# NVIDIA-Genomics-Research/GenomeWorks

Measured on AMD Instinct MI355X. Metric: cudapoa consensus GCUPS, 1024-window short-read batch (static band 256, 32 reads <= 1024 bp), higher is better.
Workload: dtype int16; 1 GPU; BASELINE configs[2]: cudapoa single-batch consensus, 1024 windows x 32 reads, backbone 960 bp, <=48 sub/24 ins/24 del, BatchConfig(1024,32,256,static_band), scores 8/-6/-8; windows_per_gpu=1024, cells_per_gpu=10990578176, parallelism=index-split x1

## Files before the change

genomeworks_amd/build.py:

```python
import hashlib
import os
import subprocess
import sys

PKG = os.path.dirname(os.path.abspath(__file__))
ROOT = os.path.dirname(PKG)
LIB = os.path.join(PKG, "lib")
ROCM = os.environ.get("ROCM_PATH", "/opt/rocm")
HIPCC = os.path.join(ROCM, "bin", "hipcc")

KERNEL_SRCS = ["csrc/gwhip_poa.hip", "csrc/gwhip_poa_part0.hip", "csrc/gwhip_poa_part1.hip", "csrc/gwhip_poa_part2.hip",
               "csrc/gwhip_poa_part3.hip", "csrc/gwhip_poa_part4.hip", "csrc/gwhip_poa_part5.hip", "csrc/gwhip_poa_part6.hip", "csrc/gwhip_poa_part7.hip", "csrc/gwhip_poa_hooks.hip", "csrc/gwhip_myers.hip", "csrc/gwhip_ukkonen.hip"]
HOST_SRCS = ["host/capi.cpp", "host/cudapoa_batch.cpp", "host/cudapoa_utils.cpp", "host/cudaaligner.cpp", "host/aligner_global.cpp", "host/device_pool.cpp",
             "host/aligner_semiglobal.cpp", "host/alignment_impl.cpp", "host/runtime.cpp", "host/logging.cpp", "host/overlap_alignment.cpp", "host/multi_device.cpp",
             "host/fasta_parser.cpp"]
EXTENDER_KERNEL_SRCS = ["extender/gwx_ungapped_xdrop.hip"]
EXTENDER_HOST_SRCS = ["extender/extender.cpp"]
SEMIGLOBAL_KERNEL_SRCS = ["semiglobal/gws_ends.hip"]
MAPPER_KERNEL_SRCS = ["mapper/gwm_mapper.hip", "mapper/gwm_postprocess.hip", "mapper/gwm_align.hip",
                      "mapper/gwm_index_cache.hip"]
MAPPER_HOST_SRCS = ["mapper/mapper.cpp", "mapper/gwm_driver.cpp", "mapper/gwm_index_batcher.cpp"]

KERNEL_FLAGS = ["--offload-arch=gfx950", "-O3", "-std=c++17", "-fPIC", "-fno-fast-math", "-ffp-contract=off",
                "-fhip-fp32-correctly-rounded-divide-sqrt"]
KERNEL_FLAGS += [f for f in os.environ.get("GW_KERNEL_EXTRA_FLAGS", "").split() if f]
HOST_FLAGS = ["-O2", "-g", "-std=c++17", "-fPIC", "-Wall", "-Wextra", "-Wno-unused-parameter",
              "-D__HIP_PLATFORM_AMD__", "-pthread"]


def _digest(paths, extra):
    h = hashlib.sha256(repr(extra).encode())
    for p in sorted(paths):
        with open(p, "rb") as f:
            h.update(p.encode())
            h.update(f.read())
    return h.hexdigest()


def kernel_source_digest():
    h = hashlib.sha256()
    base = os.path.join(PKG, "csrc")
    paths = [os.path.join(base, f) for f in os.listdir(base) if f.endswith((".hip", ".h"))] + [os.path.join(ROOT, "include", "gwhip.h")]
    for p in sorted(paths):
        with open(p, "rb") as f:
            h.update(os.path.relpath(p, ROOT).encode())
            h.update(f.read())
    return h.hexdigest()


def _deps(subdir, exts):
    out = []
    for base in (os.path.join(PKG, subdir), os.path.join(ROOT, "include")):
        for d, _, fs in os.walk(base):
            out += [os.path.join(d, f) for f in fs if f.endswith(exts)]
    return out


def _run(cmd):
    print("[build]", " ".join(cmd), flush=True)
    subprocess.run(cmd, check=True)


def _stale(target, stamp_value):
    stamp = target + ".stamp"
    if not os.path.exists(target) or not os.path.exists(stamp):
# ... 161 lines not shown
```

genomeworks_amd/csrc/gwhip_poa.hip:

```cpp
#include <hip/hip_runtime.h>

#include <cstdio>
#include <cstdlib>
#include <cstring>
#include <string>

#include "poa_device.h"
#include "poa_full_device.h"
#include "poa_graph_device.h"
#include "poa_tb_device.h"

namespace gwhip
{

#ifndef GWHIP_POA_PART
thread_local std::string g_last_error;

static int fail(hipError_t e, const char* what)
{
    g_last_error = std::string(what) + ": " + hipGetErrorString(e);
    return (int)e;
}
static int fail_msg(int code, const std::string& msg)
{
    g_last_error = msg;
    return code;
}
#endif

constexpr int kRingBytes   = 8448;
constexpr int kRowInfoLds  = 3074;
constexpr int kRowInfoBytes = kRowInfoLds * 8;
constexpr int kReadLds     = 2048;
constexpr int kCodeTileLds = 4096;
static_assert(kReadLds + kCodeTileLds >= 3072 * 2, "the incremental topsort keeps the previous order (uint16 x 3072) in the read + code-tile regions");
constexpr int kBsRingBytes   = 2048;
constexpr int kReadWinBytes  = 4096;
constexpr int kMwLds         = 768;
constexpr size_t kReservedCuLds = 128 * 1024;

struct KernelArgs
{
    gwhip_poa_config cfg;
    PoaLayout L;
    int32_t total_windows;
    const uint8_t* sequences;
    const int8_t* base_weights;
    int32_t* sequence_lengths;
    const gwhip_window_details* window_details;
    uint8_t* consensus;
    uint16_t* coverage;
    uint8_t* msa;
    uint8_t* workspace;
    uint8_t* full_scores;
    uint64_t* cells;
    uint64_t* phase_cycles;
    int32_t debug_flags;
    int32_t cons_lds_nodes;
    int32_t wide_ring_bytes;
    uint32_t* work_counters;
};

template <typename IdT>
__device__ GraphView<IdT> carve_graph(uint8_t* slab, const PoaLayout& L)
{
    GraphView<IdT> g;
    g.nodes                = slab + L.nodes;
    g.incoming_edge_count  = (uint16_t*)(slab + L.in_cnt);
    g.outgoing_edge_count  = (uint16_t*)(slab + L.out_cnt);
    g.node_alignment_count = (uint16_t*)(slab + L.aln_cnt);
    g.coverage             = (uint16_t*)(slab + L.coverage);
    g.sorted_poa           = (IdT*)(slab + L.sorted);
    g.node_id_to_pos       = (IdT*)(slab + L.pos);
    g.local_cnt            = (uint16_t*)(slab + L.local_cnt);
    g.incoming_edges       = (IdT*)(slab + L.in_edges);
    g.incoming_edge_w      = (uint16_t*)(slab + L.in_w);
    g.outgoing_edges       = (IdT*)(slab + L.out_edges);
    g.node_alignments      = (IdT*)(slab + L.aligned);
    g.cons_scores          = (int32_t*)(slab + L.cons_scores);
    g.cons_pred            = (IdT*)(slab + L.cons_pred);
    g.marks                = slab + L.marks;
    g.check                = slab + L.check;
    g.to_visit             = (IdT*)(slab + L.to_visit);
    g.out_cov              = (uint16_t*)(slab + L.out_cov);
    g.out_cov_cnt          = (uint16_t*)(slab + L.out_cov_cnt);
    g.msa_pos              = (IdT*)(slab + L.msa_pos);
    g.seq_begin            = (IdT*)(slab + L.seq_begin);
    return g;
}

template <typename ScoreT, typename IdT, typename TraceT, int BM, bool MSA, bool LDS_TABLES, int NW, int VARIANT>
__global__ __launch_bounds__(kWave * NW) void poa_window_kernel(KernelArgs a)
{
    constexpr bool DBG = VARIANT == 1 || VARIANT == 4 || VARIANT == 6;
    constexpr int PV   = VARIANT == 0 ? 0 : (VARIANT <= 2 ? 1 : 2);
    constexpr bool kFullPacked = (VARIANT == 5 || VARIANT == 6) && BM == GWHIP_FULL_BAND && LDS_TABLES && std::is_same<ScoreT, int16_t>::value;
    const int32_t debug_flags = DBG ? a.debug_flags : 0;
    extern __shared__ __attribute__((aligned(16))) uint8_t smem[];
    const int lane       = threadIdx.x & (kWave - 1);
    const int wave       = __builtin_amdgcn_readfirstlane((int)threadIdx.x >> 6);
    for (int32_t w = blockIdx.x; w < a.total_windows;)
    {
    const gwhip_poa_config& c = a.cfg;
    uint8_t* slab        = a.workspace + (size_t)w * a.L.per_window;
    GraphView<IdT> g     = carve_graph<IdT>(slab, a.L);
    const gwhip_window_details wd = a.window_details[w];
    int32_t* seq_lens    = a.sequence_lengths + wd.seq_len_buffer_offset;
    const uint8_t* sequence    = a.sequences + wd.seq_starts;
    const int8_t* base_weights = a.base_weights + wd.seq_starts;
    uint8_t* consensus   = a.consensus + (size_t)w * c.max_consensus_size;
    int32_t* alignment_graph = (int32_t*)(slab + a.L.align_graph);
    int32_t* alignment_read  = (int32_t*)(slab + a.L.align_read);

    ScoreT* ring = reinterpret_cast<ScoreT*>(smem);
    uint8_t* lds_rowinfo_region = smem + kRingBytes;
    uint8_t* lds_read_buf       = smem + kRingBytes + kRowInfoBytes;
    uint8_t* lds_code_tile      = LDS_TABLES ? smem + kRingBytes + kRowInfoBytes + kReadLds : nullptr;
    const int32_t ring_bytes    = LDS_TABLES ? kRingBytes : a.wide_ring_bytes;
    int32_t* lds_bs_ring        = LDS_TABLES ? nullptr : reinterpret_cast<int32_t*>(smem + ring_bytes);
    uint8_t* lds_read_window    = LDS_TABLES ? nullptr : smem + ring_bytes + kBsRingBytes;
    uint8_t* codes              = a.L.codes ? slab + a.L.codes : nullptr;
    constexpr bool graph_fits_lds = LDS_TABLES;
    using RowT = RowInfo<LDS_TABLES>;
    RowT* rowinfo;
    if constexpr (LDS_TABLES)
        rowinfo = reinterpret_cast<RowT*>(smem + kRingBytes);
    else
        rowinfo = reinterpret_cast<RowT*>(slab + a.L.rowinfo);

    constexpr bool TB = (BM == GWHIP_STATIC_BAND_TRACEBACK || BM == GWHIP_ADAPTIVE_BAND_TRACEBACK);
    ScoreT* scores;
    uint8_t* full_moves = nullptr;
    if (BM == GWHIP_FULL_BAND)
    {
        const size_t cell_bytes = sizeof(ScoreT) + (sizeof(ScoreT) == 2 ? 1 : 0);
        uint8_t* region         = a.full_scores + (size_t)wd.scores_offset * (size_t)c.max_nodes_per_graph * cell_bytes;
        scores                  = reinterpret_cast<ScoreT*>(region);
        if (sizeof(ScoreT) == 2) full_moves = region + (size_t)wd.scores_width * (size_t)c.max_nodes_per_graph * sizeof(ScoreT);
    }
    else
        scores = reinterpret_cast<ScoreT*>(slab + a.L.scores);
    TraceT* traceback = TB ? reinterpret_cast<TraceT*>(slab + a.L.trace) : nullptr;
    const float banded_buffer_size = __fmul_rn((float)c.max_nodes_per_graph, (float)c.matrix_sequence_dimension);
    MwArgs<ScoreT>* mw_args = nullptr;
    MwShared* mw_shared     = nullptr;
    if constexpr (NW > 1)
    {
        {
            int32_t bases = lane < (int32_t)wd.num_seqs ? seq_lens[lane] : 0;
            for (int off = 32; off > 0; off >>= 1) bases += __shfl_xor(bases, off);
            bases = __builtin_amdgcn_readfirstlane(bases);
            const int32_t level = bases >= (1 << 19) ? 3 : (bases >= (1 << 18) ? 2 : (bases >= (1 << 17) ? 1 : 0));
            if (level == 3) __builtin_amdgcn_s_setprio(3);
            else if (level == 2) __builtin_amdgcn_s_setprio(2);
            else if (level == 1) __builtin_amdgcn_s_setprio(1);
// ... 239 lines not shown
        if constexpr (kCachedSort)
        {
            const bool incr_ok = c.max_nodes_per_graph <= 131071 && !(debug_flags & (1 << 17)) &&
                                 (int64_t)a.L.scores_elems * (int64_t)sizeof(ScoreT) >= (int64_t)c.max_nodes_per_graph * 24 + 2048;
            if (status_and_count >= 0 && !c.spoa_accurate && !(debug_flags & (1 << 21)) && incr_ok)
            {
                wave_sync();
                bool done = false;
                if (!(debug_flags & (1 << 16)) && topsort_incr_cnt8_lds_bytes(status_and_count) <= ring_bytes)
                    done = topsort_kahn_incr_cnt8<IdT>(g, node_count, status_and_count, smem, reinterpret_cast<int32_t*>(scores), lane);
                if (!done) topsort_kahn_incr_hbm<IdT>(g, node_count, status_and_count, reinterpret_cast<int32_t*>(scores), lane);
                sorted_here = true;
            }
            else if (status_and_count >= 0 && !c.spoa_accurate && !(debug_flags & (1 << 21)) &&
                     (int64_t)a.L.scores_elems * (int64_t)sizeof(ScoreT) >= (int64_t)(2 * ((node_count + 63) & ~63)) * 4)
            {
                wave_sync();
                topsort_kahn_cached<IdT>(g, node_count, status_and_count, smem, reinterpret_cast<int32_t*>(scores), lane);
                sorted_here = true;
            }
        }
        if (lane == 0 && status_and_count >= 0 && !sorted_here)
        {
            const int32_t new_count = status_and_count;
            if (c.spoa_accurate)
                topsort_racon<IdT>(g, new_count, (int32_t)(uint16_t)c.max_nodes_per_graph);
            else if (!graph_fits_lds)
                topsort_kahn<IdT>(g.sorted_poa, g.node_id_to_pos, new_count, g.incoming_edge_count,
                                  g.outgoing_edges, g.outgoing_edge_count, g.local_cnt);
        }
        wave_sync();
        if (status_and_count >= 0 && !c.spoa_accurate && graph_fits_lds)
        {
            if constexpr (LDS_TABLES)
            {
                if (!(debug_flags & (1 << 21)))
                    topsort_kahn_incr_lds<IdT>(g, node_count, status_and_count, lds_rowinfo_region, smem, lds_read_buf, lane,
                                               debug_flags, pc.acc ? &pc.acc[kPhOther] : nullptr);
                else
                    topsort_kahn_lds<IdT>(g, status_and_count, lds_rowinfo_region, smem, lane, debug_flags, pc.acc ? &pc.acc[kPhOther] : nullptr);
            }
        }
        pc.tick(kPhTopsort);
        if (status_and_count < 0) break;
        node_count = status_and_count;
    }
    if (lane == 0 && a.cells) a.cells[w] = cells;
    if (DBG && lane == 0 && a.phase_cycles)
        for (int k = 0; k < kPhCount; k++) a.phase_cycles[(size_t)w * kPhCount + k] = phase_acc[k];
    if constexpr (NW > 1)
    {
        if (lane == 0) mw_args->op = 2;
        block_barrier();
        break;
    }
    else
    {
        if ((int32_t)gridDim.x >= a.total_windows || a.work_counters == nullptr) break;
        wave_sync();
        int32_t next = 0;
        if (lane == 0) next = (int32_t)gridDim.x + (int32_t)atomicAdd(a.work_counters, 1u);
        w = wave_first(next);
    }
    }
    if constexpr (NW == 1)
        if ((int32_t)gridDim.x < a.total_windows && a.work_counters != nullptr && threadIdx.x == 0)
        {
            __threadfence();
            if (atomicAdd(a.work_counters + 1, 1u) == gridDim.x - 1)
            {
                a.work_counters[0] = 0;
                a.work_counters[1] = 0;
                __threadfence();
            }
        }
}

#ifndef GWHIP_POA_PART
template <typename IdT>
__global__ __launch_bounds__(kWave) void poa_consensus_kernel(KernelArgs a)
{
    const int32_t w    = blockIdx.x;
    const gwhip_poa_config& c = a.cfg;
    uint8_t* consensus = a.consensus + (size_t)w * c.max_consensus_size;
    if (consensus[0] == kKernelError) return;
    uint8_t* slab      = a.workspace + (size_t)w * a.L.per_window;
    GraphView<IdT> g   = carve_graph<IdT>(slab, a.L);
    const int32_t n    = a.sequence_lengths[a.window_details[w].seq_len_buffer_offset];
    if (threadIdx.x == 0)
        generate_consensus<IdT>(g, n, g.cons_pred, g.cons_scores, consensus, a.coverage + (size_t)w * c.max_consensus_size,
                                c.max_consensus_size);
}

__global__ __launch_bounds__(kWave) void poa_consensus_lds_kernel(KernelArgs a)
{
    extern __shared__ __align__(16) uint8_t cons_smem[];
    const int32_t w    = blockIdx.x;
    const gwhip_poa_config& c = a.cfg;
    uint8_t* consensus = a.consensus + (size_t)w * c.max_consensus_size;
    if (consensus[0] == kKernelError) return;
    uint8_t* slab          = a.workspace + (size_t)w * a.L.per_window;
    GraphView<int16_t> g   = carve_graph<int16_t>(slab, a.L);
    const int32_t n        = a.sequence_lengths[a.window_details[w].seq_len_buffer_offset];
    if (n <= a.cons_lds_nodes)
        generate_consensus_lds<int16_t>(g, n, cons_smem, a.cons_lds_nodes, consensus, a.coverage + (size_t)w * c.max_consensus_size,
                                        c.max_consensus_size, threadIdx.x & (kWave - 1),
                                        (a.debug_flags & 16) != 0);
    else if (threadIdx.x == 0)
        generate_consensus<int16_t>(g, n, g.cons_pred, g.cons_scores, consensus, a.coverage + (size_t)w * c.max_consensus_size,
                                    c.max_consensus_size);
}

constexpr int kMsaStackEntries = 4096;

template <typename IdT>
__global__ __launch_bounds__(kWave) void poa_msa_kernel(KernelArgs a)
{
    extern __shared__ __attribute__((aligned(16))) uint8_t msa_smem[];
    __shared__ int32_t msa_length;
    const int32_t w    = blockIdx.x;
    const gwhip_poa_config& c = a.cfg;
    uint8_t* consensus = a.consensus + (size_t)w * c.max_consensus_size;
    if (consensus[0] == kKernelError) return;
    uint8_t* slab      = a.workspace + (size_t)w * a.L.per_window;
    GraphView<IdT> g   = carve_graph<IdT>(slab, a.L);
    const gwhip_window_details wd = a.window_details[w];
    const int32_t n    = a.sequence_lengths[wd.seq_len_buffer_offset];
    const int lane     = threadIdx.x & (kWave - 1);
// ... 35 lines not shown
__global__ void poa_export_graph_kernel(KernelArgs a, int32_t first_window, uint8_t* nodes, int32_t* in_edges, uint16_t* in_w,
                                        uint16_t* in_cnt, int32_t* out_edges, uint16_t* out_cnt)
{
    const int32_t w  = first_window + blockIdx.x;
    const size_t o   = blockIdx.x;
    const int32_t mn = a.cfg.max_nodes_per_graph;
    uint8_t* slab    = a.workspace + (size_t)w * a.L.per_window;
    GraphView<IdT> g = carve_graph<IdT>(slab, a.L);
    const int32_t n  = a.sequence_lengths[a.window_details[w].seq_len_buffer_offset];
    if (a.consensus[(size_t)w * a.cfg.max_consensus_size] == kKernelError) return;
    for (int32_t i = threadIdx.x; i < n && i < mn; i += blockDim.x)
    {
        nodes[o * mn + i]  = g.nodes[i];
        uint16_t ic        = g.incoming_edge_count[i];
        in_cnt[o * mn + i] = ic;
        for (int32_t e = 0; e < ic && e < kEdges; e++)
        {
            in_edges[(o * mn + i) * kEdges + e] = g.incoming_edges[(int64_t)i * kEdges + e];
            in_w[(o * mn + i) * kEdges + e]     = g.incoming_edge_w[(int64_t)i * kEdges + e];
        }
        if (out_edges && out_cnt)
        {
            uint16_t oc         = g.outgoing_edge_count[i];
            out_cnt[o * mn + i] = oc;
            for (int32_t e = 0; e < oc && e < kEdges; e++)
                out_edges[(o * mn + i) * kEdges + e] = g.outgoing_edges[(int64_t)i * kEdges + e];
        }
    }
}

#endif

#ifndef GWHIP_DEVICE_ONLY
#ifndef GWHIP_POA_PART
static size_t full_score_bytes(const gwhip_poa_config& c, int32_t windows, uint64_t sum_scores_width)
{
    if (c.band_mode != GWHIP_FULL_BAND) return 0;
    uint64_t per_window_width = (uint64_t)((c.max_sequence_size + 1 + kCellsPerLane + 3) & ~3);
    uint64_t width_sum        = sum_scores_width ? sum_scores_width : per_window_width * (uint64_t)windows;
    return (size_t)(width_sum * (uint64_t)c.max_nodes_per_graph * (c.score32 ? 4u : 3u)) + 256;
}

static bool validate(const gwhip_poa_args* args)
{
    const gwhip_poa_config& c = args->cfg;
    if (args->total_windows < 0 || c.max_nodes_per_graph <= 0 || c.max_consensus_size < 2) return false;
    if (c.band_mode < 0 || c.band_mode > GWHIP_ADAPTIVE_BAND_TRACEBACK) return false;
    if (c.band_mode != GWHIP_FULL_BAND && (c.alignment_band_width % 128 != 0 || c.alignment_band_width <= 0)) return false;
    if (!c.size32 && c.max_nodes_per_graph > 32767) return false;
    return true;
}
#endif

template <int BM, bool MSA, int VARIANT>
hipError_t launch_packed_variant(const KernelArgs& ka, dim3 grid, size_t lds, hipStream_t stream);
#if defined(GWHIP_POA_PART) && GWHIP_POA_PART >= 4
template <int BM, bool MSA, int VARIANT>
hipError_t launch_packed_variant(const KernelArgs& ka, dim3 grid, size_t lds, hipStream_t stream)
{
    hipLaunchKernelGGL((poa_window_kernel<int16_t, int16_t, int8_t, BM, MSA, true, 1, VARIANT>), grid, dim3(kWave), lds, stream, ka);
    return hipGetLastError();
}
#if GWHIP_POA_PART == 7
template hipError_t launch_packed_variant<GWHIP_FULL_BAND, false, 5>(const KernelArgs&, dim3, size_t, hipStream_t);
template hipError_t launch_packed_variant<GWHIP_FULL_BAND, true, 5>(const KernelArgs&, dim3, size_t, hipStream_t);
template hipError_t launch_packed_variant<GWHIP_FULL_BAND, false, 6>(const KernelArgs&, dim3, size_t, hipStream_t);
template hipError_t launch_packed_variant<GWHIP_FULL_BAND, true, 6>(const KernelArgs&, dim3, size_t, hipStream_t);
#elif GWHIP_POA_PART == 4 || GWHIP_POA_PART == 5
#if GWHIP_POA_PART == 4
#define GW_PACKED_VARIANTS(BM, MSA) template hipError_t launch_packed_variant<BM, MSA, 2>(const KernelArgs&, dim3, size_t, hipStream_t);
#else
#define GW_PACKED_VARIANTS(BM, MSA)                                                                       \
    template hipError_t launch_packed_variant<BM, MSA, 3>(const KernelArgs&, dim3, size_t, hipStream_t); \
    template hipError_t launch_packed_variant<BM, MSA, 4>(const KernelArgs&, dim3, size_t, hipStream_t);
#endif
GW_PACKED_VARIANTS(GWHIP_STATIC_BAND, false)
GW_PACKED_VARIANTS(GWHIP_STATIC_BAND, true)
GW_PACKED_VARIANTS(GWHIP_ADAPTIVE_BAND, false)
GW_PACKED_VARIANTS(GWHIP_ADAPTIVE_BAND, true)
#undef GW_PACKED_VARIANTS
#endif
#endif

template <typename ScoreT, typename IdT, typename TraceT, bool MSA, bool LDS_TABLES>
static hipError_t launch_window_kernel(const KernelArgs& ka_in, hipStream_t stream)
{
    KernelArgs ka = ka_in;
    constexpr size_t wide_rest = (size_t)kBsRingBytes + kReadWinBytes + kMwLds;
    ka.wide_ring_bytes = 5 * (kMaxAdaptiveBand + kRightPad) * 4;
    const size_t lds   = LDS_TABLES ? (size_t)kRingBytes + kRowInfoBytes + kReadLds + kCodeTileLds : (size_t)ka.wide_ring_bytes + wide_rest;
    dim3 grid(ka.total_windows);
    if (LDS_TABLES && ka.work_counters != nullptr)
    {
        static const int simds = [] {
            int cus = 0, dev = 0;
            (void)hipGetDevice(&dev);
            if (hipDeviceGetAttribute(&cus, hipDeviceAttributeMultiprocessorCount, dev) != hipSuccess || cus <= 0) cus = 256;
            return 4 * cus;
        }();
        if (ka.total_windows > simds) grid = dim3(simds);
    }
    if (grid.x >= (unsigned)ka.total_windows) ka.work_counters = nullptr;
#define GW_LAUNCH(BM)                                                                                              \
    {                                                                                                              \
        constexpr int NW = (!LDS_TABLES && BM == GWHIP_ADAPTIVE_BAND) ? kSkWaves : 1;                              \
        size_t lds_req = lds;                                                                                      \
        if (NW > 1)              \
        {                                                                                                          \
            lds_req            = kReservedCuLds;                                                                   \
            ka.wide_ring_bytes = (int32_t)(kReservedCuLds - wide_rest);                                            \
            (void)hipFuncSetAttribute(reinterpret_cast<const void*>(&poa_window_kernel<ScoreT, IdT, TraceT, BM, MSA, LDS_TABLES, NW, 0>), \
                                      hipFuncAttributeMaxDynamicSharedMemorySize, (int)kReservedCuLds);             \
            (void)hipFuncSetAttribute(reinterpret_cast<const void*>(&poa_window_kernel<ScoreT, IdT, TraceT, BM, MSA, LDS_TABLES, NW, 1>), \
                                      hipFuncAttributeMaxDynamicSharedMemorySize, (int)kReservedCuLds);             \
        }                                                                                                          \
        constexpr bool kHasPacked = LDS_TABLES && std::is_same<ScoreT, int16_t>::value && std::is_same<TraceT, int8_t>::value && \
                                    (BM == GWHIP_STATIC_BAND || BM == GWHIP_ADAPTIVE_BAND);                        \
        const bool debug = ka.debug_flags != 0 || ka.phase_cycles != nullptr;                                      \
        const int32_t bw = ka.cfg.alignment_band_width;                                                            \
        bool launched    = false;                                                                                  \
        if constexpr (kHasPacked)                                                                                  \
        {                                                                                                          \
            constexpr int PBM = kHasPacked ? BM : GWHIP_STATIC_BAND;                                               \
            if (bw == 384 || bw == 512)                                                                            \
            {                                                                                                      \
                hipError_t pe = debug ? launch_packed_variant<PBM, MSA, 4>(ka, grid, lds_req, stream)             \
                                      : launch_packed_variant<PBM, MSA, 3>(ka, grid, lds_req, stream);            \
                if (pe != hipSuccess) return pe;                                                                   \
                launched = true;                                                                                   \
            }                                                                                                      \
            else if (bw == 128 && !debug)                                                                          \
            {                                                                                                      \
                hipError_t pe = launch_packed_variant<PBM, MSA, 2>(ka, grid, lds_req, stream);                     \
                if (pe != hipSuccess) return pe;                                                                   \
                launched = true;                                                                                   \
            }                                                                                                      \
        }                                                                                                          \
        if constexpr (BM == GWHIP_FULL_BAND && LDS_TABLES && std::is_same<ScoreT, int16_t>::value && std::is_same<IdT, int16_t>::value && \
                      std::is_same<TraceT, int8_t>::value)                                                         \
        {                                                                                                          \
            hipError_t pe = debug ? launch_packed_variant<GWHIP_FULL_BAND, MSA, 6>(ka, grid, lds_req, stream)      \
                                  : launch_packed_variant<GWHIP_FULL_BAND, MSA, 5>(ka, grid, lds_req, stream);     \
            if (pe != hipSuccess) return pe;                                                                       \
            launched = true;                                                                                       \
        }                                                                                                          \
        if (launched) {}                                                                                           \
        else if (debug)                                                                                            \
            hipLaunchKernelGGL((poa_window_kernel<ScoreT, IdT, TraceT, BM, MSA, LDS_TABLES, NW, 1>), grid, dim3(kWave * NW), lds_req, stream, ka); \
        else                                                                                                       \
            hipLaunchKernelGGL((poa_window_kernel<ScoreT, IdT, TraceT, BM, MSA, LDS_TABLES, NW, 0>), grid, dim3(kWave * NW), lds_req, stream, ka); \
    }                                                                                                              \
    break;
    switch (ka.cfg.band_mode)
    {
    case GWHIP_FULL_BAND: GW_LAUNCH(GWHIP_FULL_BAND)
    case GWHIP_STATIC_BAND: GW_LAUNCH(GWHIP_STATIC_BAND)
    case GWHIP_ADAPTIVE_BAND: GW_LAUNCH(GWHIP_ADAPTIVE_BAND)
    case GWHIP_STATIC_BAND_TRACEBACK: GW_LAUNCH(GWHIP_STATIC_BAND_TRACEBACK)
    default: GW_LAUNCH(GWHIP_ADAPTIVE_BAND_TRACEBACK)
    }
#undef GW_LAUNCH
    return hipGetLastError();
}

template <typename ScoreT, typename IdT, typename TraceT>
hipError_t launch_msa_split(const KernelArgs& ka, hipStream_t stream)
{
    constexpr bool can_lds = sizeof(IdT) == 2;
    const bool lds = can_lds && ka.cfg.max_nodes_per_graph + 2 <= kRowInfoLds && ka.cfg.max_sequence_size + 16 <= kReadLds;
    if (ka.cfg.output_mask & 2)
    {
        if constexpr (can_lds)
            if (lds) return launch_window_kernel<ScoreT, IdT, TraceT, true, true>(ka, stream);
        return launch_window_kernel<ScoreT, IdT, TraceT, true, false>(ka, stream);
    }
    if constexpr (can_lds)
        if (lds) return launch_window_kernel<ScoreT, IdT, TraceT, false, true>(ka, stream);
    return launch_window_kernel<ScoreT, IdT, TraceT, false, false>(ka, stream);
}

#if defined(GWHIP_POA_PART) && GWHIP_POA_PART == 6
template hipError_t launch_msa_split<int16_t, int16_t, int16_t>(const KernelArgs&, hipStream_t);
#else
extern template hipError_t launch_msa_split<int16_t, int16_t, int16_t>(const KernelArgs&, hipStream_t);
#endif

template <typename ScoreT, typename IdT>
hipError_t launch_trace_split(const KernelArgs& ka, hipStream_t stream)
{
    const bool tb = ka.cfg.band_mode == GWHIP_STATIC_BAND_TRACEBACK || ka.cfg.band_mode == GWHIP_ADAPTIVE_BAND_TRACEBACK;
    if (tb && ka.cfg.trace16) return launch_msa_split<ScoreT, IdT, int16_t>(ka, stream);
    return launch_msa_split<ScoreT, IdT, int8_t>(ka, stream);
}
#ifdef GWHIP_POA_PART
#if GWHIP_POA_PART == 0
template hipError_t launch_trace_split<int32_t, int32_t>(const KernelArgs&, hipStream_t);
#elif GWHIP_POA_PART == 1
template hipError_t launch_trace_split<int32_t, int16_t>(const KernelArgs&, hipStream_t);
#elif GWHIP_POA_PART == 2
template hipError_t launch_trace_split<int16_t, int32_t>(const KernelArgs&, hipStream_t);
#elif GWHIP_POA_PART == 3
template hipError_t launch_trace_split<int16_t, int16_t>(const KernelArgs&, hipStream_t);
#endif
#else
extern template hipError_t launch_trace_split<int32_t, int32_t>(const KernelArgs&, hipStream_t);
extern template hipError_t launch_trace_split<int32_t, int16_t>(const KernelArgs&, hipStream_t);
extern template hipError_t launch_trace_split<int16_t, int32_t>(const KernelArgs&, hipStream_t);
extern template hipError_t launch_trace_split<int16_t, int16_t>(const KernelArgs&, hipStream_t);

static KernelArgs make_kernel_args(const gwhip_poa_args* args)
{
    KernelArgs ka{};
    ka.cfg             = args->cfg;
    ka.L               = make_poa_layout(args->cfg);
    ka.total_windows   = args->total_windows;
    ka.sequences       = args->sequences;
    ka.base_weights    = args->base_weights;
    ka.sequence_lengths = args->sequence_lengths;
    ka.window_details  = args->window_details;
    ka.consensus       = args->consensus;
    ka.coverage        = args->coverage;
    ka.msa             = args->msa;
    ka.workspace       = (uint8_t*)args->workspace;
    ka.full_scores     = ka.workspace + (size_t)args->total_windows * ka.L.per_window;
    ka.cells           = args->cells;
    ka.phase_cycles    = args->phase_cycles;
    ka.work_counters   = args->work_counters;
    if (const char* pg = std::getenv("GWHIP_POA_PERSISTENT"))
        if (pg[0] == '0') ka.work_counters = nullptr;
    {
        const char* dbg = std::getenv("GWHIP_DEBUG");
        ka.debug_flags  = dbg ? std::atoi(dbg) : 0;
    }
    return ka;
}
#endif

#endif
}

#if !defined(GWHIP_DEVICE_ONLY) && !defined(GWHIP_POA_PART)
using namespace gwhip;

extern "C" {

size_t gwhip_poa_workspace_bytes(const gwhip_poa_config* cfg, int32_t windows, uint64_t sum_scores_width)
// ... 152 lines not shown
```

genomeworks_amd/csrc/poa_forward_moves.h:

```cpp
#pragma once

namespace gwhip
{

constexpr int kKindShift = 60;
constexpr uint32_t kMoveHoriz = 1;

__device__ __forceinline__ uint32_t pk_mad_u16_vsv(uint32_t a, uint32_t s, uint32_t c)
{
    uint32_t d;
    asm("v_pk_mad_u16 %0, %1, %2, %3" : "=v"(d) : "v"(a), "s"(s), "v"(c));
    return d;
}
__device__ __forceinline__ uint32_t pk_mad_u16_vvs(uint32_t a, uint32_t b, uint32_t s)
{
    uint32_t d;
    asm("v_pk_mad_u16 %0, %1, %2, %3" : "=v"(d) : "v"(a), "v"(b), "s"(s));
    return d;
}
__device__ __forceinline__ void gstore_nt_u64(void* p, uint32_t lo, uint32_t hi)
{
    u32x2 v;
    v.x = lo; v.y = hi;
    __builtin_nontemporal_store(v, reinterpret_cast<u32x2*>(p));
// ... 61 lines not shown
            const int32_t node_id = cnt > 3 ? (int32_t)g.sorted_poa[r - 1] : 0;
            for (int32_t k = 0; k < cnt; k++)
                mark(k < 3 ? (int32_t)((w >> (24 + 12 * k)) & 0xfffu) : (int32_t)g.node_id_to_pos[g.incoming_edges[(int64_t)node_id * kEdges + k]] + 1);
        }
    }
    wave_sync();
}
__device__ __forceinline__ bool row_recompute_safe(uint64_t w)
{
    return ((uint32_t)(w >> kKindShift) & 7u) >= 4u || ((w >> 8) & 0x3fu) > 3u || ((w >> 15) & 0x1ffu) == 0u;
}

template <typename IdT, int BW>
__device__ __forceinline__ void banded_forward_moves(const GraphView<IdT>& g, RowInfo<true>* rowinfo, int32_t graph_count,
                                                     const uint8_t* lds_read, int16_t* scores, uint8_t* moves, uint8_t* ring,
                                                     const uint64_t* xpred, int32_t max_column, int32_t gap_score,
                                                     int32_t mismatch_score, int32_t match_score, int32_t dbg,
                                                     uint64_t* prof_acc, bool store_all = true)
{
    const bool abl       = (dbg & (1 << 14)) != 0;
    const bool st_scores = !(abl && (dbg & (1 << 26))), st_moves = !(abl && (dbg & (1 << 27)));
    const bool ab_ring = !(abl && (dbg & (1 << 20))), ab_guard = !(abl && (dbg & (1 << 19))), ab_scan = !(abl && (dbg & (1 << 18))),
               ab_moves = !(abl && (dbg & (1 << 17))), ab_rows = !(abl && (dbg & (1 << 16)));
    const int32_t ksel = prof_acc ? ((dbg >> 28) & 7) - 1 : -1;
    const bool kcount  = (dbg & (1 << 12)) != 0;
    uint64_t kacc      = 0;
    static_assert(BW == 128 || BW == 256, "band widths of the packed pass");
    constexpr int32_t band_width = BW;
    constexpr int32_t stride     = band_width + kRightPad;
    constexpr int kBandLanes     = BW / kCellsPerLane;
    const int lane               = threadIdx.x & (kWave - 1);
    const bool band_lane         = lane < kBandLanes;
    const int32_t lane4 = lane * 4, lane8 = lane * 8;
    const int32_t min_score = Limits<int16_t>::min / 2;

    const int32_t first_moved = classify_kinds(rowinfo, graph_count, lane, xpred, dbg);
    wave_sync();
    mark_score_rows<IdT>(g, rowinfo, graph_count, lane, store_all);

    const uint32_t MIN2   = pin_vgpr(pk_dup(min_score));
    const uint32_t SENT2  = pin_vgpr(pk_dup(kPkSentinel));
    const uint32_t GAP2   = pin_vgpr(pk_dup(gap_score));
    const uint32_t MAT2   = pin_vgpr(pk_dup(match_score));
    const uint32_t DIF2   = pin_vgpr(pk_dup(mismatch_score - match_score));
    const uint32_t ONE2   = pin_vgpr(0x00010001u);
    const uint32_t THREE2 = pin_vgpr(0x00030003u);
    const uint32_t NEG1   = pin_vgpr(0xffffffffu);
    const uint32_t K01 = pk_make((lane4 + 0) * gap_score, (lane4 + 1) * gap_score);
    const uint32_t K23 = pk_make((lane4 + 2) * gap_score, (lane4 + 3) * gap_score);
    const uint32_t ring_base = lds_addr(ring);
    const uint32_t read_base = lds_addr(lds_read);
    const uint32_t guard_off  = lane < 16 ? (uint32_t)(2 * BW) : (lane == 16 ? (uint32_t)-136 : (uint32_t)(120 - 16 * lane));
    const bool is_lane16      = lane == 16;
    const bool is_lane63      = lane == kBandLanes - 1;
    const uint32_t move_keep  = lane == 0 ? 0xffffff00u : 0xffffffffu;
    const uint32_t GUARD_HI_MIN = pin_vgpr(is_lane16 ? (((uint32_t)kPkSentinel & 0xffffu) | ((uint32_t)min_score << 16)) : pk_dup(kPkSentinel));
    const uint32_t S0X_MIN      = (uint32_t)min_score << 16;

    uint32_t P01 = pk_make((lane4 + 1) * gap_score, (lane4 + 2) * gap_score);
    uint32_t P23 = pk_make((lane4 + 3) * gap_score, (lane4 + 4) * gap_score);
    int32_t prev_rel0 = 0;
    uint32_t rd4  = lds_load_u32(read_base + lane4);
    uint32_t rd4n = lds_load_u32(read_base + lane4 + 4);
    uint32_t a1   = (uint32_t)lane8;
    uint32_t ga   = (a1 + guard_off) & (kPkSlotBytes - 1);
    uint8_t* const score_base = reinterpret_cast<uint8_t*>(scores) + lane8 + 2 * (1 + kRelShift);
    uint8_t* move_ptr  = moves + lane4 + (1 + kRelShift);

    if (BW == 256 || band_lane) lds_store_u64(ring_base + a1, P01, P23);
    lds_store_guard(ring_base + ga, SENT2, is_lane16 ? (((uint32_t)kPkSentinel & 0xffffu) | (0u << 16)) : SENT2);

    auto scan_row = [&](uint32_t s01, uint32_t s23, int32_t cu) {
        const uint32_t u01 = pk_sub(s01, K01), u23 = pk_sub(s23, K23);
        const uint32_t pm01 = pk_max(u01, (u01 << 16) | 0x8000u);
        const uint32_t pm23 = pk_max(u23, (u23 << 16) | 0x8000u);
        const int32_t m3    = (int32_t)pk_max(pm01, pm23) >> 16;
        const int32_t incl  = ab_scan ? wave_inclusive_max(m3) : m3;
        const int32_t excl  = max(wave_shr1(incl, cu), cu);
        const uint32_t ex2  = __builtin_amdgcn_perm((uint32_t)excl, (uint32_t)excl, 0x01000100u);
        const uint32_t m1b  = __builtin_amdgcn_perm(pm01, pm01, 0x03020302u);
        P01 = pk_add(pk_max(pm01, ex2), K01);
        P23 = pk_add(pk_max(pk_max(pm23, m1b), ex2), K23);
    };
    auto nz = [&](uint32_t a, uint32_t b) -> uint32_t { return pk_min_u16(pk_sub(a, b), ONE2); };
    auto costs = [&](uint32_t base4, uint32_t& c01, uint32_t& c23) {
        const uint32_t x   = rd4 ^ base4;
        const uint32_t x01 = __builtin_amdgcn_perm(0u, x, 0x0c010c00u);
        const uint32_t x23 = __builtin_amdgcn_perm(0u, x, 0x0c030c02u);
        c01 = pk_mad_u16(pk_min_u16(x01, ONE2), DIF2, MAT2);
        c23 = pk_mad_u16(pk_min_u16(x23, ONE2), DIF2, MAT2);
    };
    auto from_pred = [&](uint32_t s0x, uint32_t q01, uint32_t q23, uint32_t c01, uint32_t c23, uint32_t& D01, uint32_t& D23,
                         uint32_t& V01, uint32_t& V23) {
        D01 = pk_add(__builtin_amdgcn_alignbit(q01, s0x, 16), c01);
        D23 = pk_add(__builtin_amdgcn_alignbit(q23, q01, 16), c23);
        V01 = pk_add(q01, GAP2);
        V23 = pk_add(q23, GAP2);
    };
    auto store_row = [&](auto bs0_tag, int32_t r, int32_t rel0_val, uint32_t mv4, bool scores_to_hbm) {
        constexpr bool BS0 = decltype(bs0_tag)::value;
        move_ptr += stride;
        const uint32_t sbase = ring_base + (((uint32_t)r & (kPkSlots - 1)) * kPkSlotBytes);
        if (BS0 || __builtin_expect(scores_to_hbm, 0))
        {
            uint8_t* score_ptr = score_base + (uint32_t)r * (uint32_t)(stride * 2);
            if (st_scores && (BW == 256 || band_lane)) gstore_nt_u64(score_ptr, P01, P23);
            if constexpr (BS0) gstore_u16_lane0_below(score_ptr, (uint32_t)rel0_val);
// ... 96 lines not shown
            int32_t t0, t1, t2, t3;
            if (prow == r - 1) from_regs(t0, t1, t2, t3);
            else from_hbm(prow, t0, t1, t2, t3);
            if (p == 0) { s0 = t0; s1 = t1; s2 = t2; s3 = t3; }
            else { s0 = max(s0, t0); s1 = max(s1, t1); s2 = max(s2, t2); s3 = max(s3, t3); }
        }
        scan_row(pk_make(s0, s1), pk_make(s2, s3), fe + gap_score);
        uint8_t* score_ptr = score_base + (uint32_t)r * (uint32_t)(stride * 2);
        move_ptr += stride;
        const uint32_t sbase  = ring_base + (((uint32_t)r & (kPkSlots - 1)) * kPkSlotBytes);
        const uint32_t rel0pk = ((uint32_t)kPkSentinel & 0xffffu) | ((uint32_t)rel0_val << 16);
        if (BW == 256 || band_lane)
        {
            *reinterpret_cast<uint2*>(score_ptr) = make_uint2(P01, P23);
            lds_store_u64(sbase + a1, P01, P23);
        }
        lds_store_guard(sbase + ga, SENT2, is_lane16 ? rel0pk : SENT2);
        if (bs == 0) gstore_u16_lane0_below(score_ptr, (uint32_t)rel0_val);
        if (BW == 256 || band_lane) *reinterpret_cast<uint32_t*>(move_ptr) = 0u;
        prev_rel0_io = rel0_val;
    };

    auto reg_row = [&](auto bs0_tag, auto moved_tag, int32_t r, uint32_t d0, uint32_t base4, bool scores_to_hbm) {
        constexpr bool BS0   = decltype(bs0_tag)::value;
        constexpr bool MOVED = decltype(moved_tag)::value;
        uint32_t s0x, q01, q23;
        if constexpr (!MOVED)
        {
            s0x = (uint32_t)wave_shr1((int32_t)P23, BS0 ? (int32_t)((uint32_t)prev_rel0 << 16) : (int32_t)S0X_MIN);
            q01 = P01; q23 = P23;
        }
        else
        {
            s0x  = P23;
            q01  = (uint32_t)wave_shl1((int32_t)P01, (int32_t)pk_dup(kPkSentinel));
            q23  = (uint32_t)wave_shl1((int32_t)P23, (int32_t)pk_dup(kPkSentinel));
            a1   = (a1 + 8) & (kPkSlotBytes - 1);
            ga   = (ga + 8) & (kPkSlotBytes - 1);
            rd4  = rd4n;
            rd4n = lds_load_u32(read_base + (((d0 >> 3) & 0x1ffu) << 2) + lane4 + 4);
        }
        int32_t cu = min_score + 2 * gap_score, rel0_val = min_score;
        if constexpr (BS0)
        {
            rel0_val = max(min_score, prev_rel0) + gap_score;
            cu       = rel0_val + gap_score;
        }
        uint32_t c01, c23, D01, D23, V01, V23;
        costs(base4, c01, c23);
        from_pred(s0x, q01, q23, c01, c23, D01, D23, V01, V23);
        uint32_t s01 = pk_max(D01, V01), s23 = pk_max(D23, V23);
        if constexpr (MOVED)
        {
            s01 = is_lane63 ? MIN2 : s01;
            s23 = is_lane63 ? MIN2 : s23;
        }
        scan_row(s01, s23, cu);
        const uint32_t m01 = pk_mad_u16(nz(P01, D01), pk_mad_u16(nz(P01, V01), NEG1, NEG1), THREE2);
        const uint32_t m23 = pk_mad_u16(nz(P23, D23), pk_mad_u16(nz(P23, V23), NEG1, NEG1), THREE2);
        uint32_t mv4 = ab_moves ? pack_moves(m01, m23) : 0u;
        if constexpr (MOVED) mv4 = is_lane63 ? 0u : mv4;
        store_row(bs0_tag, r, rel0_val, mv4, scores_to_hbm);
    };

    auto run_rows = [&](auto bs0_tag, int32_t r_from, int32_t r_to) {
        constexpr bool BS0 = decltype(bs0_tag)::value;
        int32_t r = r_from;
        while (r <= r_to)
        {
            const int32_t r0   = r;
            uint32_t D0v, D1v;
            {
                const int32_t rr    = min(r0 + lane, graph_count);
                const uint64_t w    = rowinfo[rr].w;
                const uint32_t kind = (uint32_t)(w >> kKindShift) & 7u;
                const uint32_t cnt  = (uint32_t)(w >> 8) & 0x3fu;
                const uint32_t bs4  = (uint32_t)(w >> 15) & 0x1ffu;
                const uint32_t p0 = (uint32_t)(w >> 24) & 0xfffu, p1 = (uint32_t)(w >> 36) & 0xfffu, p2 = (uint32_t)(w >> 48) & 0xfffu;
                const uint32_t slots = (p0 & 7u) | ((p1 & 7u) << 3) | ((p2 & 7u) << 6);
                const uint32_t dists = (((uint32_t)rr - p0) & 7u) | ((((uint32_t)rr - p1) & 7u) << 3) | ((((uint32_t)rr - p2) & 7u) << 6);
                D0v = kind | (bs4 << 3) | (slots << 12) | (dists << 21) | ((cnt <= 3 ? cnt : 0u) << 30);
                D1v = ((uint32_t)w & 0xffu) * 0x01010101u;
            }
            D0v = (r0 + lane <= r_to) ? D0v : 7u;
            const uint64_t need64 = BS0 ? ~0ull : __ballot((rowinfo[min(r0 + lane, graph_count)].w & kRowScoresInHbm) != 0);
            int32_t k      = 0;
            uint32_t d0    = (uint32_t)__builtin_amdgcn_readlane((int32_t)D0v, 0);
            uint32_t base4 = (uint32_t)__builtin_amdgcn_readlane((int32_t)D1v, 0);
            uint32_t kind  = d0 & 7u;
            auto advance = [&]() {
                r++;
                k++;
                const uint32_t nd = (uint32_t)__builtin_amdgcn_readlane((int32_t)D0v, k & (kWave - 1));
                base4 = (uint32_t)__builtin_amdgcn_readlane((int32_t)D1v, k & (kWave - 1));
                d0    = k == kWave ? 7u : nd;
                kind  = d0 & 7u;
            };
            for (;;)
            {
                const uint64_t t_k0 = ksel == 0 ? clock64() : 0;
                const int32_t r_k0  = r;
                while (kind == 0)
                {
                    reg_row(bs0_tag, std::false_type{}, r, d0, base4, ((need64 >> k) & 1ull) != 0);
                    advance();
                }
                if (ksel == 0) kacc += kcount ? (uint64_t)(r - r_k0) : clock64() - t_k0;
                if (kind == 7u) break;
                const int32_t kind_now = (int32_t)min(kind, 4u);
                const uint64_t t_kx    = ksel == kind_now ? clock64() : 0;
                const bool scores_to_hbm = ((need64 >> k) & 1ull) != 0;
                if (kind == 1)
                    reg_row(bs0_tag, std::true_type{}, r, d0, base4, scores_to_hbm);
                else if (kind <= 3)
// ... 151 lines not shown
```

Measured before the change: 389.3 GCUPS.

## Split persistent work-stealing POA kernel into its own instantiation and mask lane-63 with bitwise ops

Moves the per-window body into a device function and adds a separate PERSISTENT template variant that holds the atomic work-stealing loop. The non-persistent kernel becomes a single window per block with no loop or end-of-grid counter reset. The counters are now zeroed with hipMemsetAsync before each persistent launch, replacing the in-kernel last-block reset. The lane-63 selects in the forward-moves row step become AND/OR masks on a pinned VGPR constant, aiming to avoid v_cndmask and keep the per-row lane-compare out of the inner loop. The cost is more instantiations, longer compile time and an extra memset on the stream.

```diff
diff --git a/genomeworks_amd/build.py b/genomeworks_amd/build.py
--- a/genomeworks_amd/build.py
+++ b/genomeworks_amd/build.py
@@ -10,7 +10,9 @@
 HIPCC = os.path.join(ROCM, "bin", "hipcc")
 
 KERNEL_SRCS = ["csrc/gwhip_poa.hip", "csrc/gwhip_poa_part0.hip", "csrc/gwhip_poa_part1.hip", "csrc/gwhip_poa_part2.hip",
-               "csrc/gwhip_poa_part3.hip", "csrc/gwhip_poa_part4.hip", "csrc/gwhip_poa_part5.hip", "csrc/gwhip_poa_part6.hip", "csrc/gwhip_poa_part7.hip", "csrc/gwhip_poa_hooks.hip", "csrc/gwhip_myers.hip", "csrc/gwhip_ukkonen.hip"]
+               "csrc/gwhip_poa_part3.hip", "csrc/gwhip_poa_part4.hip", "csrc/gwhip_poa_part5.hip", "csrc/gwhip_poa_part6.hip", "csrc/gwhip_poa_part7.hip",
+               "csrc/gwhip_poa_persistent0.hip", "csrc/gwhip_poa_persistent1.hip", "csrc/gwhip_poa_persistent2.hip", "csrc/gwhip_poa_persistent3.hip",
+               "csrc/gwhip_poa_persistent4.hip", "csrc/gwhip_poa_persistent5.hip", "csrc/gwhip_poa_persistent6.hip", "csrc/gwhip_poa_hooks.hip", "csrc/gwhip_myers.hip", "csrc/gwhip_ukkonen.hip"]
 HOST_SRCS = ["host/capi.cpp", "host/cudapoa_batch.cpp", "host/cudapoa_utils.cpp", "host/cudaaligner.cpp", "host/aligner_global.cpp", "host/device_pool.cpp",
              "host/aligner_semiglobal.cpp", "host/alignment_impl.cpp", "host/runtime.cpp", "host/logging.cpp", "host/overlap_alignment.cpp", "host/multi_device.cpp",
              "host/fasta_parser.cpp"]
diff --git a/genomeworks_amd/csrc/gwhip_poa.hip b/genomeworks_amd/csrc/gwhip_poa.hip
--- a/genomeworks_amd/csrc/gwhip_poa.hip
+++ b/genomeworks_amd/csrc/gwhip_poa.hip
@@ -1,5 +1,6 @@
 #include <hip/hip_runtime.h>
 
+#include <atomic>
 #include <cstdio>
 #include <cstdlib>
 #include <cstring>
@@ -90,17 +91,13 @@
 }
 
 template <typename ScoreT, typename IdT, typename TraceT, int BM, bool MSA, bool LDS_TABLES, int NW, int VARIANT>
-__global__ __launch_bounds__(kWave * NW) void poa_window_kernel(KernelArgs a)
-{
+__device__ __forceinline__ void poa_window_body(const KernelArgs& a, const int32_t w, const int lane, const int wave)
+{
+    extern __shared__ __attribute__((aligned(16))) uint8_t smem[];
     constexpr bool DBG = VARIANT == 1 || VARIANT == 4 || VARIANT == 6;
     constexpr int PV   = VARIANT == 0 ? 0 : (VARIANT <= 2 ? 1 : 2);
     constexpr bool kFullPacked = (VARIANT == 5 || VARIANT == 6) && BM == GWHIP_FULL_BAND && LDS_TABLES && std::is_same<ScoreT, int16_t>::value;
     const int32_t debug_flags = DBG ? a.debug_flags : 0;
-    extern __shared__ __attribute__((aligned(16))) uint8_t smem[];
-    const int lane       = threadIdx.x & (kWave - 1);
-    const int wave       = __builtin_amdgcn_readfirstlane((int)threadIdx.x >> 6);
-    for (int32_t w = blockIdx.x; w < a.total_windows;)
-    {
     const gwhip_poa_config& c = a.cfg;
     uint8_t* slab        = a.workspace + (size_t)w * a.L.per_window;
     GraphView<IdT> g     = carve_graph<IdT>(slab, a.L);
@@ -446,28 +443,28 @@
     {
         if (lane == 0) mw_args->op = 2;
         block_barrier();
-        break;
-    }
+    }
+}
+
+template <typename ScoreT, typename IdT, typename TraceT, int BM, bool MSA, bool LDS_TABLES, int NW, int VARIANT, bool PERSISTENT = false>
+__global__ __launch_bounds__(kWave * NW) void poa_window_kernel(KernelArgs a)
+{
+    const int lane = threadIdx.x & (kWave - 1);
+    const int wave = __builtin_amdgcn_readfirstlane((int)threadIdx.x >> 6);
+    if constexpr (!PERSISTENT)
+        poa_window_body<ScoreT, IdT, TraceT, BM, MSA, LDS_TABLES, NW, VARIANT>(a, (int32_t)blockIdx.x, lane, wave);
     else
     {
-        if ((int32_t)gridDim.x >= a.total_windows || a.work_counters == nullptr) break;
-        wave_sync();
-        int32_t next = 0;
-        if (lane == 0) next = (int32_t)gridDim.x + (int32_t)atomicAdd(a.work_counters, 1u);
-        w = wave_first(next);
-    }
-    }
-    if constexpr (NW == 1)
-        if ((int32_t)gridDim.x < a.total_windows && a.work_counters != nullptr && threadIdx.x == 0)
-        {
-            __threadfence();
-            if (atomicAdd(a.work_counters + 1, 1u) == gridDim.x - 1)
-            {
-                a.work_counters[0] = 0;
-                a.work_counters[1] = 0;
-                __threadfence();
-            }
-        }
+        static_assert(LDS_TABLES && NW == 1, "the persistent grid belongs to the single-wave LDS-table kernels");
+        for (int32_t w = blockIdx.x; w < a.total_windows;)
+        {
+            poa_window_body<ScoreT, IdT, TraceT, BM, MSA, LDS_TABLES, NW, VARIANT>(a, w, lane, wave);
+            wave_sync();
+            int32_t next = 0;
+            if (lane == 0) next = (int32_t)gridDim.x + (int32_t)atomicAdd(a.work_counters, 1u);
+            w = wave_first(next);
+        }
+    }
 }
 
 #ifndef GWHIP_POA_PART
@@ -609,12 +606,50 @@
 }
 #endif
 
+template <typename ScoreT, typename TraceT, int BM, bool MSA, int VARIANT>
+hipError_t launch_persistent(const KernelArgs& ka, dim3 grid, size_t lds, hipStream_t stream);
+#ifdef GWHIP_POA_PERSISTENT_PART
+template <typename ScoreT, typename TraceT, int BM, bool MSA, int VARIANT>
+hipError_t launch_persistent(const KernelArgs& ka, dim3 grid, size_t lds, hipStream_t stream)
+{
+    hipLaunchKernelGGL((poa_window_kernel<ScoreT, int16_t, TraceT, BM, MSA, true, 1, VARIANT, true>), grid, dim3(kWave), lds, stream, ka);
+    return hipGetLastError();
+}
+#define GW_PERSISTENT(ScoreT, TraceT, BM, VARIANT)                                                                              \
+    template hipError_t launch_persistent<ScoreT, TraceT, BM, false, VARIANT>(const KernelArgs&, dim3, size_t, hipStream_t);   \
+    template hipError_t launch_persistent<ScoreT, TraceT, BM, true, VARIANT>(const KernelArgs&, dim3, size_t, hipStream_t);
+#define GW_PERSISTENT_MODES(ScoreT, TraceT)                                                                 \
+    GW_PERSISTENT(ScoreT, TraceT, GWHIP_FULL_BAND, 0) GW_PERSISTENT(ScoreT, TraceT, GWHIP_FULL_BAND, 1)     \
+    GW_PERSISTENT(ScoreT, TraceT, GWHIP_STATIC_BAND, 0) GW_PERSISTENT(ScoreT, TraceT, GWHIP_STATIC_BAND, 1) \
+    GW_PERSISTENT(ScoreT, TraceT, GWHIP_ADAPTIVE_BAND, 0) GW_PERSISTENT(ScoreT, TraceT, GWHIP_ADAPTIVE_BAND, 1) \
+    GW_PERSISTENT(ScoreT, TraceT, GWHIP_STATIC_BAND_TRACEBACK, 0) GW_PERSISTENT(ScoreT, TraceT, GWHIP_STATIC_BAND_TRACEBACK, 1) \
+    GW_PERSISTENT(ScoreT, TraceT, GWHIP_ADAPTIVE_BAND_TRACEBACK, 0) GW_PERSISTENT(ScoreT, TraceT, GWHIP_ADAPTIVE_BAND_TRACEBACK, 1)
+#if GWHIP_POA_PERSISTENT_PART == 0
+GW_PERSISTENT_MODES(int32_t, int8_t)
+#elif GWHIP_POA_PERSISTENT_PART == 1
+GW_PERSISTENT_MODES(int32_t, int16_t)
+#elif GWHIP_POA_PERSISTENT_PART == 2
+GW_PERSISTENT_MODES(int16_t, int8_t)
+#elif GWHIP_POA_PERSISTENT_PART == 3
+GW_PERSISTENT_MODES(int16_t, int16_t)
+#elif GWHIP_POA_PERSISTENT_PART == 4
+GW_PERSISTENT(int16_t, int8_t, GWHIP_STATIC_BAND, 2) GW_PERSISTENT(int16_t, int8_t, GWHIP_ADAPTIVE_BAND, 2)
+#elif GWHIP_POA_PERSISTENT_PART == 5
+GW_PERSISTENT(int16_t, int8_t, GWHIP_STATIC_BAND, 3) GW_PERSISTENT(int16_t, int8_t, GWHIP_ADAPTIVE_BAND, 3)
+GW_PERSISTENT(int16_t, int8_t, GWHIP_STATIC_BAND, 4) GW_PERSISTENT(int16_t, int8_t, GWHIP_ADAPTIVE_BAND, 4)
+#elif GWHIP_POA_PERSISTENT_PART == 6
+GW_PERSISTENT(int16_t, int8_t, GWHIP_FULL_BAND, 5) GW_PERSISTENT(int16_t, int8_t, GWHIP_FULL_BAND, 6)
+#endif
+#undef GW_PERSISTENT_MODES
+#undef GW_PERSISTENT
+#else
 template <int BM, bool MSA, int VARIANT>
 hipError_t launch_packed_variant(const KernelArgs& ka, dim3 grid, size_t lds, hipStream_t stream);
 #if defined(GWHIP_POA_PART) && GWHIP_POA_PART >= 4
 template <int BM, bool MSA, int VARIANT>
 hipError_t launch_packed_variant(const KernelArgs& ka, dim3 grid, size_t lds, hipStream_t stream)
 {
+    if (ka.work_counters != nullptr) return launch_persistent<int16_t, int8_t, BM, MSA, VARIANT>(ka, grid, lds, stream);
     hipLaunchKernelGGL((poa_window_kernel<int16_t, int16_t, int8_t, BM, MSA, true, 1, VARIANT>), grid, dim3(kWave), lds, stream, ka);
     return hipGetLastError();
 }
@@ -639,6 +674,23 @@
 #endif
 #endif
 
+static int device_simds()
+{
+    constexpr int kMaxDevices = 64;
+    static std::atomic<int> cache[kMaxDevices];
+    int dev = 0, cus = 0;
+    if (hipGetDevice(&dev) != hipSuccess) dev = -1;
+    if (dev >= 0 && dev < kMaxDevices)
+        if (const int known = cache[dev].load(std::memory_order_relaxed)) return known;
+    if (dev < 0 || hipDeviceGetAttribute(&cus, hipDeviceAttributeMultiprocessorCount, dev) != hipSuccess || cus <= 0)
+    {
+        (void)hipGetLastError();
+        return 4 * 256;
+    }
+    if (dev < kMaxDevices) cache[dev].store(4 * cus, std::memory_order_relaxed);
+    return 4 * cus;
+}
+
 template <typename ScoreT, typename IdT, typename TraceT, bool MSA, bool LDS_TABLES>
 static hipError_t launch_window_kernel(const KernelArgs& ka_in, hipStream_t stream)
 {
@@ -649,15 +701,11 @@
     dim3 grid(ka.total_windows);
     if (LDS_TABLES && ka.work_counters != nullptr)
     {
-        static const int simds = [] {
-            int cus = 0, dev = 0;
-            (void)hipGetDevice(&dev);
-            if (hipDeviceGetAttribute(&cus, hipDeviceAttributeMultiprocessorCount, dev) != hipSuccess || cus <= 0) cus = 256;
-            return 4 * cus;
-        }();
+        const int simds = device_simds();
         if (ka.total_windows > simds) grid = dim3(simds);
     }
     if (grid.x >= (unsigned)ka.total_windows) ka.work_counters = nullptr;
+    else if (hipError_t ze = hipMemsetAsync(ka.work_counters, 0, 2 * sizeof(uint32_t), stream); ze != hipSuccess) return ze;
 #define GW_LAUNCH(BM)                                                                                              \
     {                                                                                                              \
         constexpr int NW = (!LDS_TABLES && BM == GWHIP_ADAPTIVE_BAND) ? kSkWaves : 1;                              \
@@ -702,6 +750,15 @@
             launched = true;                                                                                       \
         }                                                                                                          \
         if (launched) {}                                                                                           \
+        else if (LDS_TABLES && NW == 1 && ka.work_counters != nullptr)                                             \
+        {                                                                                                          \
+            if constexpr (LDS_TABLES && NW == 1)                                                                   \
+            {                                                                                                      \
+                hipError_t pe = debug ? launch_persistent<ScoreT, TraceT, BM, MSA, 1>(ka, grid, lds_req, stream)   \
+                                      : launch_persistent<ScoreT, TraceT, BM, MSA, 0>(ka, grid, lds_req, stream);  \
+                if (pe != hipSuccess) return pe;                                                                   \
+            }                                                                                                      \
+        }                                                                                                          \
         else if (debug)                                                                                            \
             hipLaunchKernelGGL((poa_window_kernel<ScoreT, IdT, TraceT, BM, MSA, LDS_TABLES, NW, 1>), grid, dim3(kWave * NW), lds_req, stream, ka); \
         else                                                                                                       \
@@ -749,6 +806,7 @@
     if (tb && ka.cfg.trace16) return launch_msa_split<ScoreT, IdT, int16_t>(ka, stream);
     return launch_msa_split<ScoreT, IdT, int8_t>(ka, stream);
 }
+#endif
 #ifdef GWHIP_POA_PART
 #if GWHIP_POA_PART == 0
 template hipError_t launch_trace_split<int32_t, int32_t>(const KernelArgs&, hipStream_t);
diff --git a/genomeworks_amd/csrc/gwhip_poa_persistent0.hip b/genomeworks_amd/csrc/gwhip_poa_persistent0.hip
--- /dev/null
+++ b/genomeworks_amd/csrc/gwhip_poa_persistent0.hip
@@ -0,0 +1,3 @@
+#define GWHIP_POA_PART 8
+#define GWHIP_POA_PERSISTENT_PART 0
+#include "gwhip_poa.hip"
diff --git a/genomeworks_amd/csrc/gwhip_poa_persistent1.hip b/genomeworks_amd/csrc/gwhip_poa_persistent1.hip
--- /dev/null
+++ b/genomeworks_amd/csrc/gwhip_poa_persistent1.hip
@@ -0,0 +1,3 @@
+#define GWHIP_POA_PART 8
+#define GWHIP_POA_PERSISTENT_PART 1
+#include "gwhip_poa.hip"
diff --git a/genomeworks_amd/csrc/gwhip_poa_persistent2.hip b/genomeworks_amd/csrc/gwhip_poa_persistent2.hip
--- /dev/null
+++ b/genomeworks_amd/csrc/gwhip_poa_persistent2.hip
@@ -0,0 +1,3 @@
+#define GWHIP_POA_PART 8
+#define GWHIP_POA_PERSISTENT_PART 2
+#include "gwhip_poa.hip"
diff --git a/genomeworks_amd/csrc/gwhip_poa_persistent3.hip b/genomeworks_amd/csrc/gwhip_poa_persistent3.hip
--- /dev/null
+++ b/genomeworks_amd/csrc/gwhip_poa_persistent3.hip
@@ -0,0 +1,3 @@
+#define GWHIP_POA_PART 8
+#define GWHIP_POA_PERSISTENT_PART 3
+#include "gwhip_poa.hip"
diff --git a/genomeworks_amd/csrc/gwhip_poa_persistent4.hip b/genomeworks_amd/csrc/gwhip_poa_persistent4.hip
--- /dev/null
+++ b/genomeworks_amd/csrc/gwhip_poa_persistent4.hip
@@ -0,0 +1,3 @@
+#define GWHIP_POA_PART 8
+#define GWHIP_POA_PERSISTENT_PART 4
+#include "gwhip_poa.hip"
diff --git a/genomeworks_amd/csrc/gwhip_poa_persistent5.hip b/genomeworks_amd/csrc/gwhip_poa_persistent5.hip
--- /dev/null
+++ b/genomeworks_amd/csrc/gwhip_poa_persistent5.hip
@@ -0,0 +1,3 @@
+#define GWHIP_POA_PART 8
+#define GWHIP_POA_PERSISTENT_PART 5
+#include "gwhip_poa.hip"
diff --git a/genomeworks_amd/csrc/gwhip_poa_persistent6.hip b/genomeworks_amd/csrc/gwhip_poa_persistent6.hip
--- /dev/null
+++ b/genomeworks_amd/csrc/gwhip_poa_persistent6.hip
@@ -0,0 +1,3 @@
+#define GWHIP_POA_PART 8
+#define GWHIP_POA_PERSISTENT_PART 6
+#include "gwhip_poa.hip"
diff --git a/genomeworks_amd/csrc/poa_forward_moves.h b/genomeworks_amd/csrc/poa_forward_moves.h
--- a/genomeworks_amd/csrc/poa_forward_moves.h
+++ b/genomeworks_amd/csrc/poa_forward_moves.h
@@ -137,7 +137,7 @@
     const uint32_t read_base = lds_addr(lds_read);
     const uint32_t guard_off  = lane < 16 ? (uint32_t)(2 * BW) : (lane == 16 ? (uint32_t)-136 : (uint32_t)(120 - 16 * lane));
     const bool is_lane16      = lane == 16;
-    const bool is_lane63      = lane == kBandLanes - 1;
+    const uint32_t KEEP63     = pin_vgpr(lane == kBandLanes - 1 ? 0u : 0xffffffffu);
     const uint32_t move_keep  = lane == 0 ? 0xffffff00u : 0xffffffffu;
     const uint32_t GUARD_HI_MIN = pin_vgpr(is_lane16 ? (((uint32_t)kPkSentinel & 0xffffu) | ((uint32_t)min_score << 16)) : pk_dup(kPkSentinel));
     const uint32_t S0X_MIN      = (uint32_t)min_score << 16;
@@ -340,14 +340,14 @@
         uint32_t s01 = pk_max(D01, V01), s23 = pk_max(D23, V23);
         if constexpr (MOVED)
         {
-            s01 = is_lane63 ? MIN2 : s01;
-            s23 = is_lane63 ? MIN2 : s23;
+            s01 = (s01 & KEEP63) | (MIN2 & ~KEEP63);
+            s23 = (s23 & KEEP63) | (MIN2 & ~KEEP63);
         }
         scan_row(s01, s23, cu);
         const uint32_t m01 = pk_mad_u16(nz(P01, D01), pk_mad_u16(nz(P01, V01), NEG1, NEG1), THREE2);
         const uint32_t m23 = pk_mad_u16(nz(P23, D23), pk_mad_u16(nz(P23, V23), NEG1, NEG1), THREE2);
         uint32_t mv4 = ab_moves ? pack_moves(m01, m23) : 0u;
-        if constexpr (MOVED) mv4 = is_lane63 ? 0u : mv4;
+        if constexpr (MOVED) mv4 &= KEEP63;
         store_row(bs0_tag, r, rel0_val, mv4, scores_to_hbm);
     };
 
```

Result: no change. 390.4 GCUPS, median of 6 (+0.3%).
